# gaurav00700/Selfsupervised-NVSF

Hardware: AMD Instinct MI355X
Metric: rendered rays/sec (LiDAR+cam) (higher is better)
Workload: dtype f16; 1 GPU; C2: KITTI-360 seq-1908-shaped frame per GPU, uniform sampling, static hash field; num_rays=4096, num_rays_lidar=4096, num_steps=768, hash_grid=L16 F2 T2^19 base16 max2048, sigma_mlp=32-64-16, heads=lidar 2x(87-64-64-1), rgb 31-64-64-3, parallelism=frame-sharded x1, no collective

## Files before the change

### selfsupervised-nvsf_amd/csrc/common.h

```cpp
#pragma once
#include <hip/hip_runtime.h>
#include <stdint.h>

#define NVSF_API extern "C" __attribute__((visibility("default")))

enum : int {
    NVSF_OK = 0,
    NVSF_ERR_INVALID_ARG = -1,
    NVSF_ERR_UNSUPPORTED = -2,
};

#define REQUIRE(cond) do { if (!(cond)) return NVSF_ERR_INVALID_ARG; } while (0)

constexpr int kWave = 64;

static inline int nvsf_launch_status() {
    hipError_t e = hipGetLastError();
    return e == hipSuccess ? NVSF_OK : (int)e;
}

static inline unsigned cdiv(unsigned long long a, unsigned b) { return (unsigned)((a + b - 1) / b); }

enum NvsfVariantKey : int {
    kVarMarch = 0,
    kVarPlanesFwd,
    kVarPlanesBwd,
    kVarHashgridFwd,
    kVarHashgridBwd,
    kVarHash4dBwd,
    kVarSlicePlan,
    kVarRenderTail,
    kVarMarchSkew,
    kVarMlpBwd,
    kVarLevelKinds,
    kVarCornerShare,
    kVarCount
};
int nvsf_variant(int key);
int nvsf_cu_count();

__device__ __forceinline__ int lane_id() { return (int)(threadIdx.x & 63); }

__device__ __forceinline__ uint32_t lane_swap(uint32_t v) {
    return (uint32_t)__builtin_amdgcn_mov_dpp((int)v, 0xB1 , 0xF, 0xF, true);
}
__device__ __forceinline__ float lane_swap_f(float v) { return __builtin_bit_cast(float, lane_swap(__builtin_bit_cast(uint32_t, v))); }

template <typename T>
__device__ __forceinline__ T wave_sum(T v) {
#pragma unroll
    for (int o = 32; o > 0; o >>= 1) v += __shfl_xor(v, o, 64);
    return v;
}

__device__ __forceinline__ float wave_scan_add(float v) {
    const int l = lane_id();
#pragma unroll
    for (int o = 1; o < 64; o <<= 1) {
        float u = __shfl_up(v, o, 64);
        if (l >= o) v += u;
    }
    return v;
}
__device__ __forceinline__ float wave_scan_mul(float v) {
    const int l = lane_id();
#pragma unroll
    for (int o = 1; o < 64; o <<= 1) {
        float u = __shfl_up(v, o, 64);
        if (l >= o) v *= u;
    }
    return v;
}
__device__ __forceinline__ uint32_t wave_scan_add_u32(uint32_t v) {
    const int l = lane_id();
#pragma unroll
    for (int o = 1; o < 64; o <<= 1) {
        uint32_t u = __shfl_up(v, o, 64);
        if (l >= o) v += u;
    }
    return v;
}

__device__ __forceinline__ uint32_t wave_scan_max_u32(uint32_t v) {
#define NVSF_DPP_MAX(ctrl, row_mask)                                                                                        \
    {                                                                                                                      \
        const uint32_t u = (uint32_t)__builtin_amdgcn_update_dpp(0, (int)v, ctrl, row_mask, 0xF, false);                   \
        v = u > v ? u : v;                                                                                                 \
    }
    NVSF_DPP_MAX(0x111, 0xF)
    NVSF_DPP_MAX(0x112, 0xF)
    NVSF_DPP_MAX(0x114, 0xF)
    NVSF_DPP_MAX(0x118, 0xF)
    NVSF_DPP_MAX(0x142, 0xA)
    NVSF_DPP_MAX(0x143, 0xC)
#undef NVSF_DPP_MAX
    return v;
}
```

### selfsupervised-nvsf_amd/csrc/fused_field.hip

```cpp
#include "hashgrid_device.h"
#include "mlp_device.h"
#include "encodings_device.h"
#include "march_device.h"
#pragma clang diagnostic ignored "-Wpass-failed"
#include <stdlib.h>

namespace {
constexpr int kBlock = 256;
constexpr int kWavesPerBlock = kBlock / kWave;

struct RayBatch {
    const float* rays_o;
    const float* rays_d;
    const float* nears;
    const float* fars;
    const float* lin;
    const float* noise;
    float lo[3], hi[3];
    float inv_extent;
    float bound;
    uint32_t N, T;
};

__device__ __forceinline__ float sample_z(const RayBatch& rb, float near, float range, float lin, const float* noise) {
// ... 50 lines not shown
        const float near = rb.nears[n], range = rb.fars[n] - near;
        float x[3];
        const float z = sample_point(rb, rb.rays_o + 3 * (size_t)n, rb.rays_d + 3 * (size_t)n, near, range, rb.lin[i], rb.noise + s, x);
        half8_t xf;
#pragma unroll
        for (int q = 0; q < kLevelsPerGroup; ++q) {
            const int l = g * kLevelsPerGroup + q;
            float acc[F];
            encode_level<3, F>(x, table, meta.scale[l], meta.res[l], meta.offset[l], meta.offset[l + 1] - meta.offset[l], acc);
#pragma unroll
            for (int f = 0; f < F; ++f) xf[q * F + f] = (_Float16)acc[f];
        }
        float4_t acc1[kHidTiles];
#pragma unroll
        for (int t = 0; t < kHidTiles; ++t) {
            const float4_t zero = {0, 0, 0, 0};
            acc1[t] = mfma16(w0[t], xf, zero);
        }
        half8_t h[kHidSteps];
        pack_hidden(acc1, h);
        const float4_t o = wout.apply(h);
        if (in_range) {
            half4_t ov;
            ov[0] = (_Float16)o[0]; ov[1] = (_Float16)o[1]; ov[2] = (_Float16)o[2]; ov[3] = (_Float16)o[3];
            if (g == 3) {
                z_vals[s] = z;
                sigmas[s] = expf(o[3]);
                ov[3] = (_Float16)1.0f;
            }
            *reinterpret_cast<half4_t*>(geo + s * 16 + 4 * g) = ov;
        }
    }
}

template <int F>
struct LaneLevels {
    static constexpr int Q = 8 / F;
    float scale[Q];
    uint32_t res[Q], res2[Q], boff[Q], rows[Q];
};

__device__ __forceinline__ void fma_entry(float w, uint32_t raw, float& a0, float& a1) {
    asm("v_fma_mix_f32 %0, %1, %2, %0 op_sel_hi:[0,1,0]" : "+v"(a0) : "v"(w), "v"(raw));
    asm("v_fma_mix_f32 %0, %1, %2, %0 op_sel:[0,1,0] op_sel_hi:[0,1,0]" : "+v"(a1) : "v"(w), "v"(raw));
}

template <int F>
__device__ __forceinline__ uint32_t gather_raw(__amdgpu_buffer_rsrc_t rsrc, uint32_t byte_off);
template <>
__device__ __forceinline__ uint32_t gather_raw<2>(__amdgpu_buffer_rsrc_t rsrc, uint32_t byte_off) {
    return __builtin_amdgcn_raw_buffer_load_b32(rsrc, byte_off, 0, 0);
}
typedef uint32_t entry4_t __attribute__((ext_vector_type(2)));
template <int F> struct EntryOf { typedef uint32_t type; };
template <> struct EntryOf<4> { typedef entry4_t type; };
template <>
__device__ __forceinline__ uint32_t gather_raw<4>(__amdgpu_buffer_rsrc_t, uint32_t) = delete;
__device__ __forceinline__ entry4_t gather_raw4(__amdgpu_buffer_rsrc_t rsrc, uint32_t byte_off) {
    return __builtin_amdgcn_raw_buffer_load_b64(rsrc, byte_off, 0, 0);
}

template <int F>
struct DensityCtx {
    static constexpr int Q = 8 / F;
    LaneLevels<F> lv;
    half8_t w0[kHidTiles];
    OutLayerW wout;
    __amdgpu_buffer_rsrc_t rsrc;
    uint32_t first_hashed;
    int g;
    const uint4* lds_lv;
    uint32_t share_mask;
    uint32_t* share_lds;
};

template <int N>
__device__ __forceinline__ uint32_t row_lane(uint32_t v) {
    return (uint32_t)__builtin_amdgcn_update_dpp(0, (int)v, 0x150 + N, 0xF, 0xF, false);
}

constexpr uint32_t kFirstHashedC2 = 5;
constexpr float kShareLambdaMax = 2.0f;
constexpr int kShareWords = 2 * kWave;
template <int F, int QG, bool LDS_LV = false, int FH = -1, bool SHARE = false>
__device__ __forceinline__ half8_t density_encode(const DensityCtx<F>& cx, const float (&x)[3]) {
    constexpr int Q = 8 / F;
    static_assert(!SHARE || (F == 2 && QG == Q), "the shared form exchanges one dword per lane and runs behind the gathers of all groups");
    LaneLevels<F> lv_local;
    if constexpr (LDS_LV) {
        uint32_t again = 0;
        asm volatile("" : "+v"(again));
#pragma unroll
        for (int q = 0; q < Q; ++q) {
            const uint4 v = cx.lds_lv[4 * q + again];
            lv_local.scale[q] = __builtin_bit_cast(float, v.x);
            lv_local.res[q] = v.y;
            lv_local.res2[q] = v.y * v.y;
            lv_local.boff[q] = v.z;
            lv_local.rows[q] = v.w;
        }
    }
    const LaneLevels<F>& lv = LDS_LV ? lv_local : cx.lv;
    const uint32_t first_hashed = FH >= 0 ? (uint32_t)FH : cx.first_hashed;
    const int g = cx.g;
    half8_t xf;
#pragma unroll
    for (int q0 = 0; q0 < Q; q0 += QG) {
    float frac[Q][3];
    typename EntryOf<F>::type raw[Q][8];
    bool shared[2] = {false, false};
    uint32_t share_sel[2] = {0u, 0u}, share_one[2] = {0u, 0u};
#pragma unroll
    for (int q = q0; q < q0 + QG; ++q) {
        uint32_t c[3];
#pragma unroll
        for (int d = 0; d < 3; ++d) {
            const float pos = fmaf(lv.scale[q], x[d], 0.5f);
            const float fl = floorf(pos);
            frac[q][d] = pos - fl;
            c[d] = (uint32_t)(int32_t)fl;
        }
        const bool all_dense = (uint32_t)(4 * q + 3) < first_hashed, all_hashed = (uint32_t)(4 * q) >= first_hashed;
        if constexpr (SHARE) {
            if (q < 2 && ((cx.share_mask >> q) & 1u)) {
                uint32_t a[3], b[3];
#pragma unroll
                for (int d = 0; d < 3; ++d) {
                    a[d] = row_lane<0>(c[d]);
                    b[d] = row_lane<15>(c[d]);
                }
                const bool in_a = c[0] == a[0] && c[1] == a[1] && c[2] == a[2], in_b = c[0] == b[0] && c[1] == b[1] && c[2] == b[2];
                share_sel[q] = in_a ? 0u : 8u;
                shared[q] = __ballot(!(in_a || in_b)) == 0;
                if (shared[q]) {
                    const uint32_t col = (uint32_t)lane_id() & 15u;
                    const bool of_a = col < 8u;
                    const uint32_t cc[3] = {(of_a ? a[0] : b[0]) + (col & 1u), (of_a ? a[1] : b[1]) + ((col >> 1) & 1u), (of_a ? a[2] : b[2]) + ((col >> 2) & 1u)};
                    uint32_t v = 0;
                    if (all_dense || !all_hashed) {
                        v = cc[0] + cc[1] * lv.res[q] + cc[2] * lv.res2[q];
                        v = v >= lv.rows[q] ? v - lv.rows[q] : v;
                    }
                    if (all_hashed || !all_dense) {
                        const uint32_t h = (cc[0] ^ (cc[1] * 2654435761u) ^ (cc[2] * 805459861u)) & (lv.rows[q] - 1u);
                        v = (all_hashed || (uint32_t)(4 * q + g) >= first_hashed) ? h : v;
                    }
                    share_one[q] = gather_raw<2>(cx.rsrc, lv.boff[q] + v * (uint32_t)(F * sizeof(_Float16)));
                }
            }
        }
        if (!SHARE || q >= 2 || !shared[q]) {
        uint32_t idx[8];
        if (all_dense || !all_hashed) {
            const uint32_t b00 = c[0] + c[1] * lv.res[q] + c[2] * lv.res2[q];
            const uint32_t b10 = b00 + lv.res[q], b01 = b00 + lv.res2[q], b11 = b10 + lv.res2[q];
            const uint32_t base[4] = {b00, b10, b01, b11};
#pragma unroll
            for (int k = 0; k < 8; ++k) {
                uint32_t v = base[k >> 1] + (uint32_t)(k & 1);
                v = v >= lv.rows[q] ? v - lv.rows[q] : v;
                idx[k] = v;
            }
        }
        if (all_hashed || !all_dense) {
            const uint32_t hy0 = c[1] * 2654435761u, hy1 = hy0 + 2654435761u;
            const uint32_t hz0 = c[2] * 805459861u, hz1 = hz0 + 805459861u;
            const uint32_t yz[4] = {hy0 ^ hz0, hy1 ^ hz0, hy0 ^ hz1, hy1 ^ hz1};
            const uint32_t mask = lv.rows[q] - 1u;
            const bool lane_hashed = (uint32_t)(4 * q + g) >= first_hashed;
#pragma unroll
            for (int k = 0; k < 8; ++k) {
                const uint32_t v = ((c[0] + (uint32_t)(k & 1)) ^ yz[k >> 1]) & mask;
                idx[k] = (all_hashed || lane_hashed) ? v : idx[k];
            }
        }
#pragma unroll
        for (int k = 0; k < 8; ++k) {
            if constexpr (F == 2) raw[q][k] = gather_raw<2>(cx.rsrc, lv.boff[q] + idx[k] * (uint32_t)(F * sizeof(_Float16)));
            else raw[q][k] = gather_raw4(cx.rsrc, lv.boff[q] + idx[k] * (uint32_t)(F * sizeof(_Float16)));
        }
        }
    }
    auto blend = [&](int q, const typename EntryOf<F>::type (&r)[8]) {
        const float fx = frac[q][0], fy = frac[q][1], fz = frac[q][2];
        const float wx[2] = {1.0f - fx, fx}, wy[2] = {1.0f - fy, fy}, wz[2] = {1.0f - fz, fz};
        if constexpr (F == 2) {
            float a0 = 0.0f, a1 = 0.0f;
#pragma unroll
            for (int k = 0; k < 8; ++k) {
                const float w = (wx[k & 1] * wy[(k >> 1) & 1]) * wz[k >> 2];
                fma_entry(w, r[k], a0, a1);
            }
            xf[q * F] = (_Float16)a0;
            xf[q * F + 1] = (_Float16)a1;
        } else {
            float a0 = 0.0f, a1 = 0.0f, a2 = 0.0f, a3 = 0.0f;
#pragma unroll
            for (int k = 0; k < 8; ++k) {
                const float w = (wx[k & 1] * wy[(k >> 1) & 1]) * wz[k >> 2];
                fma_entry(w, r[k][0], a0, a1);
                fma_entry(w, r[k][1], a2, a3);
            }
            xf[q * F] = (_Float16)a0;
            xf[q * F + 1] = (_Float16)a1;
            xf[q * F + 2] = (_Float16)a2;
            xf[q * F + 3] = (_Float16)a3;
        }
    };
    if constexpr (SHARE) {
#pragma unroll
        for (int q = 0; q < 2; ++q) {
            if (shared[q]) {
                uint32_t* slot = cx.share_lds + q * kWave;
                slot[lane_id()] = share_one[q];
                const uint4* cell = reinterpret_cast<const uint4*>(slot + 16 * g + share_sel[q]);
                const uint4 lo = cell[0], hi = cell[1];
                const uint32_t r[8] = {lo.x, lo.y, lo.z, lo.w, hi.x, hi.y, hi.z, hi.w};
                blend(q, r);
            } else {
                blend(q, raw[q]);
            }
        }
    }
#pragma unroll
    for (int q = (SHARE ? 2 : q0); q < q0 + QG; ++q) blend(q, raw[q]);
    }
    return xf;
}

template <int F, int QG>
__device__ __forceinline__ float4_t density_eval(const DensityCtx<F>& cx, const float (&x)[3]) {
    const half8_t xf = density_encode<F, QG>(cx, x);
    float4_t acc1[kHidTiles];
#pragma unroll
    for (int t = 0; t < kHidTiles; ++t) {
        const float4_t zero = {0, 0, 0, 0};
        acc1[t] = mfma16(cx.w0[t], xf, zero);
    }
    half8_t h[kHidSteps];
    pack_hidden(acc1, h);
    return cx.wout.apply(h);
}

struct TrainOut {
    float* x01;
    _Float16* feat;
    float* h32;
    uint32_t* tile;
};

__device__ __forceinline__ void store_h32(float* __restrict__ h32, unsigned long long s, int lane, int g, float o0, float o1, float o2, float o3, bool ok) {
    const int from = (lane + 48) & 63;
    const float prev = __int_as_float(__builtin_amdgcn_ds_bpermute(from << 2, __float_as_int(o3)));
    if (ok) *reinterpret_cast<float4*>(h32 + s * 16 + 4 * g) = make_float4(prev, o0, o1, o2);
}

constexpr int kTrPitch = 20;
constexpr int kTrWords = 16 * kTrPitch;
__device__ __forceinline__ void store_feat_row(_Float16* __restrict__ feat, unsigned long long s, int lane, int g, const uint4& p, bool ok,
                                               uint32_t* tile) {
    uint32_t* row = tile + (lane & 15) * kTrPitch;
    row[g] = p.x; row[4 + g] = p.y; row[8 + g] = p.z; row[12 + g] = p.w;
    const uint4 mine = *reinterpret_cast<const uint4*>(row + 4 * g);
    if (ok) *reinterpret_cast<uint4*>(feat + s * 32 + 8 * g) = mine;
}

__device__ __forceinline__ void store_feat_row_swap(_Float16* __restrict__ feat, unsigned long long s, int g, const uint4& p, bool ok) {
    const auto a = __builtin_amdgcn_permlane16_swap(p.x, p.y, false, false);
    const auto b = __builtin_amdgcn_permlane16_swap(p.z, p.w, false, false);
    const auto lo = __builtin_amdgcn_permlane32_swap(a[0], b[0], false, false);
    const auto hi = __builtin_amdgcn_permlane32_swap(a[1], b[1], false, false);
    if (ok) *reinterpret_cast<uint4*>(feat + s * 32 + 8 * g) = make_uint4(lo[0], hi[0], lo[1], hi[1]);
}

template <int F, int QG, bool TRAIN = false>
__device__ __forceinline__ void density_tile(const DensityCtx<F>& cx, const float (&x)[3], float z, unsigned long long s, bool in_range,
                                             float* __restrict__ z_vals, float* __restrict__ sigmas, _Float16* __restrict__ geo,
                                             const TrainOut* tr = nullptr) {
    const int g = cx.g;
    float4_t o;
    if constexpr (TRAIN) {
        const half8_t xf = density_encode<F, QG>(cx, x);
        float4_t acc1[kHidTiles];
#pragma unroll
        for (int t = 0; t < kHidTiles; ++t) {
            const float4_t zero = {0, 0, 0, 0};
            acc1[t] = mfma16(cx.w0[t], xf, zero);
        }
        half8_t h[kHidSteps];
        pack_hidden(acc1, h);
        o = cx.wout.apply(h);
        const int lane = lane_id();
        store_feat_row(tr->feat, s, lane, g, __builtin_bit_cast(uint4, xf), in_range, tr->tile);
        store_h32(tr->h32, s, lane, g, o[0], o[1], o[2], o[3], in_range);
        if (in_range && g == 0) { tr->x01[3 * s] = x[0]; tr->x01[3 * s + 1] = x[1]; tr->x01[3 * s + 2] = x[2]; }
    } else {
        o = density_eval<F, QG>(cx, x);
    }
    if (in_range) {
        half4_t ov;
        ov[0] = (_Float16)o[0]; ov[1] = (_Float16)o[1]; ov[2] = (_Float16)o[2]; ov[3] = (_Float16)o[3];
        if (g == 3) {
            z_vals[s] = z;
            sigmas[s] = expf(o[3]);
            ov[3] = (_Float16)1.0f;
        }
        *reinterpret_cast<half4_t*>(geo + s * 16 + 4 * g) = ov;
    }
}

// ... 88 lines not shown
    float scale;
    uint32_t res, res2, boff, rows;
    bool hashed;
};

template <int F>
__device__ __forceinline__ void slice_issue(const SliceLevel<F>& lv, __amdgpu_buffer_rsrc_t rsrc, const float (&x)[3], float (&frac)[3],
                                            uint32_t (&raw)[8]) {
    uint32_t c[3];
#pragma unroll
    for (int d = 0; d < 3; ++d) {
        const float pos = fmaf(lv.scale, x[d], 0.5f);
        const float fl = floorf(pos);
        frac[d] = pos - fl;
        c[d] = (uint32_t)(int32_t)fl;
    }
    uint32_t idx[8];
    if (!lv.hashed) {
        const uint32_t b00 = c[0] + c[1] * lv.res + c[2] * lv.res2;
        const uint32_t b10 = b00 + lv.res, b01 = b00 + lv.res2, b11 = b10 + lv.res2;
        const uint32_t base[4] = {b00, b10, b01, b11};
#pragma unroll
        for (int k = 0; k < 8; ++k) {
            uint32_t v = base[k >> 1] + (uint32_t)(k & 1);
            idx[k] = v >= lv.rows ? v - lv.rows : v;
        }
    } else {
        const uint32_t hy0 = c[1] * 2654435761u, hy1 = hy0 + 2654435761u;
        const uint32_t hz0 = c[2] * 805459861u, hz1 = hz0 + 805459861u;
        const uint32_t yz[4] = {hy0 ^ hz0, hy1 ^ hz0, hy0 ^ hz1, hy1 ^ hz1};
        const uint32_t mask = lv.rows - 1u;
#pragma unroll
        for (int k = 0; k < 8; ++k) idx[k] = ((c[0] + (uint32_t)(k & 1)) ^ yz[k >> 1]) & mask;
    }
#pragma unroll
    for (int k = 0; k < 8; ++k) raw[k] = gather_raw<F>(rsrc, lv.boff + idx[k] * (uint32_t)(F * sizeof(_Float16)));
}

__device__ __forceinline__ uint32_t slice_blend(const float (&frac)[3], const uint32_t (&raw)[8]) {
    const float fx = frac[0], fy = frac[1], fz = frac[2];
    const float wx[2] = {1.0f - fx, fx}, wy[2] = {1.0f - fy, fy}, wz[2] = {1.0f - fz, fz};
    float a0 = 0.0f, a1 = 0.0f;
#pragma unroll
    for (int k = 0; k < 8; ++k) {
        const float w = (wx[k & 1] * wy[(k >> 1) & 1]) * wz[k >> 2];
        fma_entry(w, raw[k], a0, a1);
    }
    h2_t o;
    o[0] = (_Float16)a0;
    o[1] = (_Float16)a1;
    return __builtin_bit_cast(uint32_t, o);
}

template <int F>
__device__ __forceinline__ void slice_issue_half(const SliceLevel<F>& lv, __amdgpu_buffer_rsrc_t rsrc, const float (&x)[3], uint32_t xb,
                                                 float (&frac)[3], uint32_t (&raw)[4]) {
    uint32_t c[3];
#pragma unroll
    for (int d = 0; d < 3; ++d) {
        const float pos = fmaf(lv.scale, x[d], 0.5f);
        const float fl = floorf(pos);
        frac[d] = pos - fl;
        c[d] = (uint32_t)(int32_t)fl;
    }
    uint32_t idx[4];
    if (!lv.hashed) {
        const uint32_t b00 = c[0] + c[1] * lv.res + c[2] * lv.res2;
        const uint32_t base[4] = {b00, b00 + lv.res, b00 + lv.res2, b00 + lv.res + lv.res2};
#pragma unroll
        for (int p = 0; p < 4; ++p) {
            const uint32_t v = base[p] + xb;
            idx[p] = v >= lv.rows ? v - lv.rows : v;
        }
    } else {
        const uint32_t hy0 = c[1] * 2654435761u, hy1 = hy0 + 2654435761u;
        const uint32_t hz0 = c[2] * 805459861u, hz1 = hz0 + 805459861u;
        const uint32_t yz[4] = {hy0 ^ hz0, hy1 ^ hz0, hy0 ^ hz1, hy1 ^ hz1};
        const uint32_t mask = lv.rows - 1u;
#pragma unroll
        for (int p = 0; p < 4; ++p) idx[p] = ((c[0] + xb) ^ yz[p]) & mask;
    }
#pragma unroll
    for (int p = 0; p < 4; ++p) raw[p] = gather_raw<F>(rsrc, lv.boff + idx[p] * (uint32_t)(F * sizeof(_Float16)));
}

constexpr int kPlanItems = 3;
struct SlicePlan {
    uint32_t n[8];
    uint32_t slice[8][kPlanItems], begin[8][kPlanItems], end[8][kPlanItems];
};

struct EncodeUnit {
    uint32_t s, n;
    bool in_range;
    float near, far, lin, noise, o[3], d[3];
};

template <bool UNIFORM_RAY>
__device__ __forceinline__ EncodeUnit fetch_unit(const RayBatch& rb, uint32_t M, uint32_t half_lane, uint32_t unit, uint32_t n_u, uint32_t i_u) {
    EncodeUnit u;
    const uint32_t s_raw = unit * 32u + half_lane;
    uint32_t i;
    if constexpr (UNIFORM_RAY) {
        u.in_range = true;
        u.s = s_raw;
        u.n = n_u;
        i = i_u + half_lane;
    } else {
        u.in_range = s_raw < M;
        u.s = u.in_range ? s_raw : M - 1u;
        u.n = u.s / rb.T;
        i = u.s - u.n * rb.T;
    }
    u.near = rb.nears[u.n];
    u.far = rb.fars[u.n];
    u.lin = rb.lin[i];
    u.noise = rb.noise ? rb.noise[u.s] : 0.5f;
    load_ray(rb, u.n, u.o, u.d);
    return u;
}

template <bool UNIFORM_RAY>
struct UnitCursor {
    uint32_t ray = 0, first = 0, d_ray = 0, d_first = 0;
    __device__ __forceinline__ UnitCursor(uint32_t wave, uint32_t wave_count, uint32_t T) {
        if constexpr (UNIFORM_RAY) {
            ray = (wave * 32u) / T;
            first = wave * 32u - ray * T;
            d_ray = (wave_count * 32u) / T;
            d_first = wave_count * 32u - d_ray * T;
        }
    }
    __device__ __forceinline__ void advance(uint32_t T) {
        if constexpr (UNIFORM_RAY) {
            ray += d_ray;
            first += d_first;
            if (first >= T) {
                first -= T;
                ray += 1u;
            }
        }
    }
};

template <int F, bool UNIFORM_RAY>
__global__ __launch_bounds__(kBlock) __attribute__((amdgpu_waves_per_eu(8, 8))) void k_encode_sliced_pairs(RayBatch rb, const _Float16* __restrict__ table, uint32_t table_bytes,
                                                                GridMeta meta, uint32_t L, uint32_t first_hashed, uint32_t M,
                                                                float* __restrict__ z_vals, uint2* __restrict__ feat, SlicePlan plan,
                                                                float* __restrict__ x01 = nullptr) {
    static_assert(F == 2, "F = 2 only");
    const uint32_t group = blockIdx.x & 7u, sb = blockIdx.x >> 3, n_sb = gridDim.x >> 3;
    for (uint32_t item = 0; item < plan.n[group]; ++item) {
    const uint32_t slice = plan.slice[group][item], unit_begin = plan.begin[group][item], unit_end = plan.end[group][item];
    const uint32_t grp = slice >> 1;
    const uint32_t lvl[2] = {(slice & 1u) ? grp + 4u : grp, (slice & 1u) ? grp + 8u : grp + 12u};
    SliceLevel<F> lv[2];
#pragma unroll
    for (int a = 0; a < 2; ++a) {
        const uint32_t l = lvl[a];
        lv[a].scale = meta.scale[l];
        lv[a].res = meta.res[l];
        lv[a].res2 = meta.res[l] * meta.res[l];
        lv[a].boff = meta.offset[l] * (uint32_t)(F * sizeof(_Float16));
        lv[a].rows = meta.offset[l + 1] - meta.offset[l];
        lv[a].hashed = l >= first_hashed;
    }
// ... 637 lines not shown
            c[0] = sigmoid_f32(oa[0]); c[1] = sigmoid_f32(oa[1]); c[2] = sigmoid_f32(oa[2]);
        }
#pragma unroll
        for (int i = 0; i < 16; ++i) {
            if ((uint32_t)i < cnt && alive) {
                const float s_i = readlane_f32(sigma, 48 + i);
                const float dt_i = readlane_f32(sdt, i), d1_i = readlane_f32(sd1, i);
                const float alpha = 1.0f - expf(-s_i * dt_i);
                const float T = 1.0f - ws;
                const float w = alpha * T;
                ws += w;
                t_comp += d1_i;
                dep += w * t_comp;
#pragma unroll
                for (int k = 0; k < 3; ++k) col[k] += w * readlane_f32(c[k], i);
                if (T < T_thresh) alive = false;
            }
        }
        total += cnt;
        if (cnt < 16u) alive = false;
    }
    if (lane == 0) {
        weights_sum[n] = ws;
        depth[n] = dep;
        if constexpr (LIDAR) {
            image[2 * (size_t)n] = col[0];
            image[2 * (size_t)n + 1] = col[1];
        } else {
            const float rest = 1.0f - ws;
            image[3 * (size_t)n] = col[0] + rest * bg0;
            image[3 * (size_t)n + 1] = col[1] + rest * bg1;
            image[3 * (size_t)n + 2] = col[2] + rest * bg2;
        }
    }
}

template <int N>
__device__ __forceinline__ float row_shr(float old, float v) {
    static_assert(N >= 1 && N <= 15, "row_shr:1..15");
    return __builtin_bit_cast(float, __builtin_amdgcn_update_dpp(__builtin_bit_cast(int, old), __builtin_bit_cast(int, v), 0x110 + N, 0xF, 0xF, false));
}

__device__ __forceinline__ float row_shl1(float old, float v) {
    return __builtin_bit_cast(float, __builtin_amdgcn_update_dpp(__builtin_bit_cast(int, old), __builtin_bit_cast(int, v), 0x101, 0xF, 0xF, false));
}

__device__ __forceinline__ float row_first(float v) {
    return __builtin_bit_cast(float, __builtin_amdgcn_update_dpp(0, __builtin_bit_cast(int, v), 0x150, 0xF, 0xF, false));
}

__device__ __forceinline__ float row16_scan_mul(float v) {
    v *= row_shr<1>(1.0f, v);
    v *= row_shr<2>(1.0f, v);
    v *= row_shr<4>(1.0f, v);
    v *= row_shr<8>(1.0f, v);
    return v;
}

template <int C>
__device__ __forceinline__ void store_ray(int lane, float ws, float dp, float (&img)[C], float bg0, float bg1, float bg2, int use_bg,
                                          float* __restrict__ weights_sum, float* __restrict__ depth, float* __restrict__ image) {
    ws = wave_sum(ws);
    dp = wave_sum(dp);
#pragma unroll
    for (int k = 0; k < C; ++k) img[k] = wave_sum(img[k]);
    if (lane == 0) {
        *weights_sum = ws;
        *depth = dp;
        const float bg[3] = {bg0, bg1, bg2};
        const float rest = use_bg ? 1.0f - ws : 0.0f;
#pragma unroll
        for (int k = 0; k < C; ++k) image[k] = use_bg ? img[k] + rest * bg[k] : img[k];
    }
}

struct RenderTrainOut {
    float* x01;
    _Float16* feat;
    _Float16* geo;
    float* sigma;
    float* rgb;
};

template <bool LIDAR, bool FROM_FEATURES, bool TRAIN = false, int FH = -1>
__global__ __launch_bounds__(kBlock) __attribute__((amdgpu_waves_per_eu(4, 4))) void k_render_uniform(
    RayBatch rb, const _Float16* __restrict__ table, uint32_t table_bytes, GridMeta meta, uint32_t first_hashed,
    const uint2* __restrict__ feat, const _Float16* __restrict__ w_sigma, const _Float16* __restrict__ w_a, const _Float16* __restrict__ w_b,
    float k_scale, float w_thresh, float bg0, float bg1, float bg2, int use_bg, float* __restrict__ z_vals, float* __restrict__ weights,
    float* __restrict__ weights_sum, float* __restrict__ depth, float* __restrict__ image, float share_thresh = -1.0f,
    RenderTrainOut rt = RenderTrainOut()) {
    using FR = OccFrags<LIDAR>;
    constexpr int F = 2;
    constexpr int IN_STEPS = FR::IN_STEPS;
    constexpr int C = LIDAR ? 2 : 3;
    __shared__ uint4 s_lv[kMaxLevels];
    __shared__ half8_t s_frag[FR::kCount * kWave];
    __shared__ float4_t s_pre[kWavesPerBlock * FR::kPre];
    __shared__ __attribute__((aligned(16))) uint32_t s_share[FROM_FEATURES ? 1 : kWavesPerBlock * kShareWords];
    fill_level_table<F>(s_lv, meta);
    const int lane = lane_id(), g = lane >> 4, c = lane & 15;
    for (int f = (int)(threadIdx.x >> 6); f < FR::kCount; f += kWavesPerBlock) s_frag[f * kWave + lane] = occ_fragment<LIDAR>(f, lane, w_sigma, w_a, w_b);
    __syncthreads();
    const uint32_t n = __builtin_amdgcn_readfirstlane(blockIdx.x * kWavesPerBlock + (threadIdx.x >> 6));
    if (n >= rb.N) return;
    const half8_t* frag = s_frag + lane;
    const uint32_t T = rb.T;
    const size_t M = (size_t)rb.N * T;

    DensityCtx<F> cx;
    if constexpr (!FROM_FEATURES) {
        cx.g = g;
        cx.first_hashed = first_hashed;
        cx.lds_lv = s_lv + g;
        cx.rsrc = __builtin_amdgcn_make_buffer_rsrc(const_cast<_Float16*>(table), 0, (int)table_bytes, 0x00020000);
    }
    const float rd0 = rb.rays_d[3 * (size_t)n], rd1 = rb.rays_d[3 * (size_t)n + 1], rd2 = rb.rays_d[3 * (size_t)n + 2];
    const float d0 = (rd0 + 1.0f) / 2.0f, d1 = (rd1 + 1.0f) / 2.0f, d2 = (rd2 + 1.0f) / 2.0f;
    half8_t xf[IN_STEPS];
    encode_ray_direction<LIDAR>(d0, d1, d2, g, xf);
    const GeoRoute<LIDAR> route(g, lane & 15);
    float4_t* pre = s_pre + (threadIdx.x >> 6) * FR::kPre;
    ray_head_constants<LIDAR>(xf, w_a, w_b, lane, pre);

    const float near = rb.nears[n], range = rb.fars[n] - near;
    const float sample_dist = range / (float)T;
    const float ro[3] = {rb.rays_o[3 * (size_t)n], rb.rays_o[3 * (size_t)n + 1], rb.rays_o[3 * (size_t)n + 2]}, rd[3] = {rd0, rd1, rd2};
    if constexpr (!FROM_FEATURES) {
        const float step1 = (sample_dist * rb.inv_extent) * ((fabsf(rd0) + fabsf(rd1)) + fabsf(rd2));
        const uint32_t m = ((16.0f * meta.scale[3]) * step1 <= share_thresh ? 1u : 0u) | ((16.0f * meta.scale[7]) * step1 <= share_thresh ? 2u : 0u);
        cx.share_mask = __builtin_amdgcn_readfirstlane(m);
        cx.share_lds = s_share + (threadIdx.x >> 6) * kShareWords;
    }
    const size_t row0 = (size_t)n * T;
    float carry = 1.0f, ws = 0.0f, dp = 0.0f, img[C];
#pragma unroll
    for (int k = 0; k < C; ++k) img[k] = 0.0f;
    float lin_cur = 0.0f, lin_nxt = 0.0f, nz_cur = 0.5f, nz_nxt = 0.5f;
    auto request = [&](uint32_t i0) {
        const uint32_t i = i0 + (uint32_t)c;
        const uint32_t ic = i < T ? i : T - 1u, in = ic + 1u < T ? ic + 1u : ic;
        lin_cur = rb.lin[ic];
        lin_nxt = rb.lin[in];
        if (rb.noise) {
            nz_cur = rb.noise[row0 + ic];
            nz_nxt = rb.noise[row0 + in];
        }
    };
    if constexpr (!FROM_FEATURES) request(0u);
    for (uint32_t i0 = 0; i0 < T; i0 += 16) {
        const uint32_t i = i0 + (uint32_t)c;
        const bool valid = i < T;
        const uint32_t ic = valid ? i : T - 1u;
        const size_t s = row0 + ic;
        float z, z_next;
        half8_t feat8;
        if constexpr (FROM_FEATURES) {
            z = z_vals[s];
            z_next = ic + 1u < T ? z_vals[s + 1] : z;
            const uint2 p0 = feat[(size_t)(2 * g) * M + s], p1 = feat[(size_t)(2 * g + 1) * M + s];
            typedef uint32_t u4_t __attribute__((ext_vector_type(4)));
            const u4_t packed = {p0.x, p1.x, p1.y, p0.y};
            feat8 = __builtin_bit_cast(half8_t, packed);
        } else {
            z = sample_z(rb, near, range, lin_cur, &nz_cur);
            z_next = sample_z(rb, near, range, lin_nxt, &nz_nxt);
            if (i0 + 16u < T) request(i0 + 16u);
            float x[3];
            sample_x01(rb, ro, rd, z, x);
            feat8 = density_encode<F, 4, true, FH, true>(cx, x);
            if constexpr (TRAIN) {
                if (g == 0 && valid) { rt.x01[3 * s] = x[0]; rt.x01[3 * s + 1] = x[1]; rt.x01[3 * s + 2] = x[2]; }
            }
        }
        if constexpr (TRAIN) store_feat_row_swap(rt.feat, s, g, __builtin_bit_cast(uint4, feat8), valid);
        const float4_t o = sigma_tile<LIDAR>(frag, feat8);
        const float delta = (i + 1u < T) ? z_next - z : sample_dist;
        float alpha = 0.0f;
        if (g == 3 && valid) alpha = 1.0f - expf(-delta * k_scale * expf(o[3]));
        const float om = (g == 3 && valid) ? (1.0f - alpha + 1e-15f) : 1.0f;
        const float incl = row16_scan_mul(om);
        const float excl = row_shr<1>(1.0f, incl);
        const float w = alpha * (carry * excl);
        carry = carry * readlane_f32(incl, 63);
        if (g == 3 && valid) {
            weights[s] = w;
            if constexpr (!FROM_FEATURES) z_vals[s] = z;
            if constexpr (TRAIN) rt.sigma[s] = expf(o[3]);
        }
        ws += w;
        dp += w * z;
        const float w0 = __shfl(w, 48 + c, 64);
        const bool on = w0 > w_thresh;
        float cr[C];
#pragma unroll
        for (int k = 0; k < C; ++k) cr[k] = 0.0f;
        if constexpr (TRAIN) {
            if (valid) *reinterpret_cast<uint2*>(rt.geo + s * 16 + 4 * g) = make_uint2(pack_h2(o[0], o[1]), pack_h2(o[2], g == 3 ? 1.0f : o[3]));
        }
        if (__ballot(w > w_thresh)) {
            const half8_t x_last = route.apply(o, g, 0, xf[IN_STEPS - 1]);
            const float4_t oa = head_tile<LIDAR>(frag, pre, g, 0, x_last);
            if constexpr (LIDAR) {
                const float4_t ob = head_tile<LIDAR>(frag, pre, g, 1, x_last);
                if (g == 0 && on) {
                    cr[0] = sigmoid_f32(oa[0]);
                    cr[1] = sigmoid_f32(ob[0]);
                    img[0] += w0 * cr[0];
                    img[1] += w0 * cr[1];
                }
            } else {
                if (g == 0 && on) {
#pragma unroll
                    for (int k = 0; k < 3; ++k) {
                        cr[k] = sigmoid_f32(oa[k]);
                        img[k] += w0 * cr[k];
                    }
                }
            }
        }
        if constexpr (TRAIN) {
            if (g == 0 && valid) {
#pragma unroll
                for (int k = 0; k < C; ++k) rt.rgb[s * C + k] = cr[k];
            }
        }
    }
    store_ray<C>(lane, ws, dp, img, bg0, bg1, bg2, use_bg, weights_sum + n, depth + n, image + (size_t)n * C);
}

template <bool LIDAR, bool TRAIN = false>
__global__ __launch_bounds__(kBlock) __attribute__((amdgpu_waves_per_eu(4, 4))) void k_render_tail2(
    RayBatch rb, const uint2* __restrict__ feat, const _Float16* __restrict__ w_sigma, const _Float16* __restrict__ w_a,
    const _Float16* __restrict__ w_b, float k_scale, float w_thresh, float bg0, float bg1, float bg2, int use_bg,
    const float* __restrict__ z_vals, float* __restrict__ weights, float* __restrict__ weights_sum, float* __restrict__ depth,
    float* __restrict__ image, RenderTrainOut rt = RenderTrainOut()) {
    using FR = OccFrags<LIDAR>;
    constexpr int IN_STEPS = FR::IN_STEPS;
    constexpr int C = LIDAR ? 2 : 3;
    constexpr int kOut1 = FR::kCount;
    __shared__ half8_t s_frag[(FR::kCount + kHidSteps) * kWave];
    __shared__ float4_t s_pre[kWavesPerBlock * FR::kPre];
    const int lane = lane_id(), g = lane >> 4, c = lane & 15;
    for (int f = (int)(threadIdx.x >> 6); f < FR::kCount + kHidSteps; f += kWavesPerBlock)
        s_frag[f * kWave + lane] = f < FR::kCount ? occ_fragment<LIDAR>(f, lane, w_sigma, w_a, w_b) : load_w_chained(w_sigma + kHidden * 32, 0, f - FR::kCount, lane, 5);
    __syncthreads();
    const uint32_t n = __builtin_amdgcn_readfirstlane(blockIdx.x * kWavesPerBlock + (threadIdx.x >> 6));
    if (n >= rb.N) return;
    const half8_t* frag = s_frag + lane;
    const uint32_t T = rb.T;
    const size_t M = (size_t)rb.N * T;

    const float rd0 = rb.rays_d[3 * (size_t)n], rd1 = rb.rays_d[3 * (size_t)n + 1], rd2 = rb.rays_d[3 * (size_t)n + 2];
// ... 319 lines not shown
    if (N == 0) return NVSF_OK;
    REQUIRE(T > 0 && weights && geo_f16 && rays_d && head_a_weights_f16 && image);
    REQUIRE(!lidar || head_b_weights_f16);
    REQUIRE(!h_bg_color || weights_sum);
    REQUIRE((reinterpret_cast<uintptr_t>(geo_f16) & 15u) == 0 && (reinterpret_cast<uintptr_t>(head_a_weights_f16) & 15u) == 0 &&
            (reinterpret_cast<uintptr_t>(head_b_weights_f16) & 15u) == 0);
    const _Float16* gp = reinterpret_cast<const _Float16*>(geo_f16);
    const _Float16* wa = reinterpret_cast<const _Float16*>(head_a_weights_f16);
    const _Float16* wb = reinterpret_cast<const _Float16*>(head_b_weights_f16);
    const float b0 = h_bg_color ? h_bg_color[0] : 0.0f, b1 = h_bg_color ? h_bg_color[1] : 0.0f,
                b2 = (h_bg_color && !lidar) ? h_bg_color[2] : 0.0f;
    const dim3 grid(cdiv(N, kWavesPerBlock)), block(kBlock);
    if (lidar)
        hipLaunchKernelGGL(k_heads_uniform<true>, dim3(grid.x, 2), block, 0, stream, weights, gp, rays_d, weights_sum, wa, wb, N, T, w_thresh, b0,
                           b1, b2, h_bg_color ? 1 : 0, image);
    else
        hipLaunchKernelGGL(k_heads_uniform<false>, grid, block, 0, stream, weights, gp, rays_d, weights_sum, wa, wb, N, T, w_thresh,
                           b0, b1, b2, h_bg_color ? 1 : 0, image);
    return nvsf_launch_status();
}

NVSF_API int nvsf_render_occupancy_fwd(const float* rays_o, const float* rays_d, const float* nears, const float* fars,
                                       const uint8_t* grid, float bound, float dt_gamma, uint32_t max_steps, uint32_t C, uint32_t H,
                                       uint32_t N, const void* table_f16, uint32_t L, uint32_t F, const float* h_scales,
                                       const uint32_t* h_res, const uint32_t* h_offsets, const void* sigma_weights_f16, int lidar,
                                       const void* head_a_weights_f16, const void* head_b_weights_f16, float density_scale,
                                       float T_thresh, const float* h_bg_color, float* weights_sum, float* depth, float* image,
                                       hipStream_t stream) {
    if (N == 0) return NVSF_OK;
    REQUIRE(rays_o && rays_d && nears && fars && grid && table_f16 && sigma_weights_f16 && head_a_weights_f16 && weights_sum && depth && image);
    REQUIRE(!lidar || head_b_weights_f16);
    REQUIRE(bound > 0.0f && C >= 1 && C <= 8 && H >= 2 && H <= 1024 && max_steps >= 1);
    REQUIRE((reinterpret_cast<uintptr_t>(table_f16) & 15u) == 0 && (reinterpret_cast<uintptr_t>(sigma_weights_f16) & 15u) == 0 &&
            (reinterpret_cast<uintptr_t>(head_a_weights_f16) & 15u) == 0 && (reinterpret_cast<uintptr_t>(head_b_weights_f16) & 15u) == 0);
    if ((F != 2 && F != 4) || L * F != 32) return NVSF_ERR_UNSUPPORTED;
    GridInfo gi;
    const int st = classify_grid(gi, L, F, h_scales, h_res, h_offsets);
    if (st != NVSF_OK) return st;
    if (!gi.dense_first || gi.table_bytes >= (1ull << 31)) return NVSF_ERR_UNSUPPORTED;
    OccRays rr;
    rr.rays_o = rays_o; rr.rays_d = rays_d; rr.nears = nears; rr.fars = fars; rr.grid = grid;
    rr.bound = bound; rr.dt_gamma = dt_gamma; rr.max_steps = max_steps; rr.C = C; rr.H = H; rr.N = N;
    const FieldParams w(table_f16, sigma_weights_f16, head_a_weights_f16, head_b_weights_f16, h_bg_color);
    const dim3 grid_dim(cdiv(N, kWavesPerBlock)), block(kBlock);
#define LAUNCH_OCC(LD, FF, FH)                                                                                                            \
    hipLaunchKernelGGL((k_render_occupancy_lds<LD, FF, FH>), grid_dim, block, 0, stream, rr, w.table, (uint32_t)gi.table_bytes, gi.meta,       \
                       gi.first_hashed, w.sigma, w.head_a, w.head_b, density_scale, T_thresh, w.bg[0], w.bg[1], w.bg[2], weights_sum, depth, \
                       image)
    const bool c2_grid = F == 2 && gi.first_hashed == kFirstHashedC2 && nvsf_variant(kVarLevelKinds) == 0;
    if (lidar) { if (c2_grid) LAUNCH_OCC(true, 2, (int)kFirstHashedC2); else if (F == 2) LAUNCH_OCC(true, 2, -1); else LAUNCH_OCC(true, 4, -1); }
    else { if (c2_grid) LAUNCH_OCC(false, 2, (int)kFirstHashedC2); else if (F == 2) LAUNCH_OCC(false, 2, -1); else LAUNCH_OCC(false, 4, -1); }
#undef LAUNCH_OCC
    return nvsf_launch_status();
}

static int render_uniform_impl(const float* rays_o, const float* rays_d, const float* nears, const float* fars, const float* lin,
                               const float* noise, const float* h_aabb, float bound, uint32_t N, uint32_t T, const void* table_f16,
                               uint32_t L, uint32_t F, const float* h_scales, const uint32_t* h_res, const uint32_t* h_offsets,
                               const void* sigma_weights_f16, int lidar, const void* head_a_weights_f16,
                               const void* head_b_weights_f16, float k_scale, float w_thresh, const float* h_bg_color,
                               const void* feat_scratch, float* z_vals, float* weights, float* weights_sum, float* depth, float* image,
                               hipStream_t stream, const RenderTrainOut* train) {
    if (N == 0 || T == 0) return NVSF_OK;
    REQUIRE(rays_o && rays_d && nears && fars && h_aabb && table_f16 && sigma_weights_f16 && head_a_weights_f16);
    REQUIRE(z_vals && weights && weights_sum && depth && image && (feat_scratch || lin));
    REQUIRE(!lidar || head_b_weights_f16);
    REQUIRE(bound > 0.0f);
    REQUIRE((reinterpret_cast<uintptr_t>(table_f16) & 15u) == 0 && (reinterpret_cast<uintptr_t>(sigma_weights_f16) & 15u) == 0 &&
            (reinterpret_cast<uintptr_t>(head_a_weights_f16) & 15u) == 0 && (reinterpret_cast<uintptr_t>(head_b_weights_f16) & 15u) == 0 &&
            (reinterpret_cast<uintptr_t>(feat_scratch) & 15u) == 0);
    if (!((F == 2 && L == 16) || (F == 4 && L == 8 && feat_scratch))) return NVSF_ERR_UNSUPPORTED;
    GridInfo gi;
    const int st = classify_grid(gi, L, F, h_scales, h_res, h_offsets);
    if (st != NVSF_OK) return st;
    if (!gi.dense_first || gi.table_bytes >= (1ull << 31)) return NVSF_ERR_UNSUPPORTED;
    const RayBatch rb = make_ray_batch(rays_o, rays_d, nears, fars, lin, noise, h_aabb, bound, N, T);
    const FieldParams w(table_f16, sigma_weights_f16, head_a_weights_f16, head_b_weights_f16, h_bg_color);
    const uint2* fp = reinterpret_cast<const uint2*>(feat_scratch);
    const RenderTrainOut rt = train ? *train : RenderTrainOut();
    const int use_bg = (h_bg_color && !lidar) ? 1 : 0;
    const dim3 grid_dim(cdiv(N, kWavesPerBlock)), block(kBlock);
    const int cs = nvsf_variant(kVarCornerShare);
    const float share_thresh = cs == 1 ? -1.0f : cs == 2 ? INFINITY : kShareLambdaMax;
#define LAUNCH_RU_FH(LD, FF, FH)                                                                                                      \
    do {                                                                                                                              \
        if (train)                                                                                                                    \
            hipLaunchKernelGGL((k_render_uniform<LD, FF, true, FH>), grid_dim, block, 0, stream, rb, w.table, (uint32_t)gi.table_bytes, gi.meta, \
                               gi.first_hashed, fp, w.sigma, w.head_a, w.head_b, k_scale, w_thresh, w.bg[0], w.bg[1], w.bg[2], use_bg, z_vals,   \
                               weights, weights_sum, depth, image, share_thresh, rt);                                                               \
        else                                                                                                                          \
            hipLaunchKernelGGL((k_render_uniform<LD, FF, false, FH>), grid_dim, block, 0, stream, rb, w.table, (uint32_t)gi.table_bytes, gi.meta, \
                               gi.first_hashed, fp, w.sigma, w.head_a, w.head_b, k_scale, w_thresh, w.bg[0], w.bg[1], w.bg[2], use_bg, z_vals,    \
                               weights, weights_sum, depth, image, share_thresh, rt);                                                               \
    } while (0)
#define LAUNCH_RU(LD, FF)                                                                                                             \
    do {                                                                                                                              \
        if (!FF && gi.first_hashed == kFirstHashedC2 && nvsf_variant(kVarLevelKinds) == 0) LAUNCH_RU_FH(LD, FF, (FF ? -1 : (int)kFirstHashedC2)); \
        else LAUNCH_RU_FH(LD, FF, -1);                                                                                                \
    } while (0)
#define LAUNCH_TAIL(LD)                                                                                                               \
    do {                                                                                                                              \
        if (train)                                                                                                                    \
            hipLaunchKernelGGL((k_render_tail2<LD, true>), grid_dim, block, 0, stream, rb, fp, w.sigma, w.head_a, w.head_b, k_scale, w_thresh, \
                               w.bg[0], w.bg[1], w.bg[2], use_bg, z_vals, weights, weights_sum, depth, image, rt);                    \
        else                                                                                                                          \
            hipLaunchKernelGGL((k_render_tail2<LD, false>), grid_dim, block, 0, stream, rb, fp, w.sigma, w.head_a, w.head_b, k_scale, w_thresh, \
                               w.bg[0], w.bg[1], w.bg[2], use_bg, z_vals, weights, weights_sum, depth, image, rt);                    \
    } while (0)
    const bool tail2 = nvsf_variant(kVarRenderTail) == 0;
    if (lidar) { if (fp) { if (tail2) LAUNCH_TAIL(true); else LAUNCH_RU(true, true); } else LAUNCH_RU(true, false); }
    else { if (fp) { if (tail2) LAUNCH_TAIL(false); else LAUNCH_RU(false, true); } else LAUNCH_RU(false, false); }
#undef LAUNCH_TAIL
#undef LAUNCH_RU
#undef LAUNCH_RU_FH
    return nvsf_launch_status();
}

NVSF_API int nvsf_render_uniform_fwd(const float* rays_o, const float* rays_d, const float* nears, const float* fars, const float* lin,
                                     const float* noise, const float* h_aabb, float bound, uint32_t N, uint32_t T, const void* table_f16,
                                     uint32_t L, uint32_t F, const float* h_scales, const uint32_t* h_res, const uint32_t* h_offsets,
                                     const void* sigma_weights_f16, int lidar, const void* head_a_weights_f16,
                                     const void* head_b_weights_f16, float k_scale, float w_thresh, const float* h_bg_color,
                                     const void* feat_scratch, float* z_vals, float* weights, float* weights_sum, float* depth, float* image,
                                     hipStream_t stream) {
    return render_uniform_impl(rays_o, rays_d, nears, fars, lin, noise, h_aabb, bound, N, T, table_f16, L, F, h_scales, h_res, h_offsets,
                               sigma_weights_f16, lidar, head_a_weights_f16, head_b_weights_f16, k_scale, w_thresh, h_bg_color, feat_scratch,
                               z_vals, weights, weights_sum, depth, image, stream, nullptr);
}

NVSF_API int nvsf_render_uniform_train_fwd(const float* rays_o, const float* rays_d, const float* nears, const float* fars, const float* lin,
                                           const float* noise, const float* h_aabb, float bound, uint32_t N, uint32_t T,
                                           const void* table_f16, uint32_t L, uint32_t F, const float* h_scales, const uint32_t* h_res,
                                           const uint32_t* h_offsets, const void* sigma_weights_f16, int lidar,
                                           const void* head_a_weights_f16, const void* head_b_weights_f16, float k_scale, float w_thresh,
                                           const float* h_bg_color, void* feat_scratch, float* z_vals, float* weights, float* weights_sum,
                                           float* depth, float* image, float* x01, void* feat_rows_f16, void* geo_f16, float* sigmas,
                                           float* rgbs, hipStream_t stream) {
    if (N == 0 || T == 0) return NVSF_OK;
    REQUIRE(x01 && feat_rows_f16 && geo_f16 && sigmas && rgbs && lin);
    REQUIRE((reinterpret_cast<uintptr_t>(feat_rows_f16) & 15u) == 0 && (reinterpret_cast<uintptr_t>(geo_f16) & 15u) == 0);
    RenderTrainOut rt;
    rt.x01 = x01; rt.feat = reinterpret_cast<_Float16*>(feat_rows_f16); rt.geo = reinterpret_cast<_Float16*>(geo_f16);
    rt.sigma = sigmas; rt.rgb = rgbs;
    if (feat_scratch) {
        TrainOut tr;
        tr.x01 = x01; tr.feat = rt.feat; tr.h32 = nullptr; tr.tile = nullptr;
        const int st = density_uniform_impl(rays_o, rays_d, nears, fars, lin, noise, h_aabb, bound, N, T, table_f16, L, F, h_scales, h_res, h_offsets,
                                            sigma_weights_f16, z_vals, sigmas, geo_f16, feat_scratch, 1u, stream, &tr);
        if (st != NVSF_OK) return st;
    }
    return render_uniform_impl(rays_o, rays_d, nears, fars, lin, noise, h_aabb, bound, N, T, table_f16, L, F, h_scales, h_res, h_offsets,
                               sigma_weights_f16, lidar, head_a_weights_f16, head_b_weights_f16, k_scale, w_thresh, h_bg_color, feat_scratch,
                               z_vals, weights, weights_sum, depth, image, stream, &rt);
}
```

### selfsupervised-nvsf_amd/csrc/version.hip

```cpp
#include "common.h"
#include <string.h>
NVSF_API const char* nvsf_version(void) { return "nvsf_hip 0.1.0 gfx950"; }

#ifndef NVSF_CSRC_DIGEST_ALL
#define NVSF_CSRC_DIGEST_ALL "unknown_________"
#endif
#ifndef NVSF_CSRC_DIGEST_RENDER
#define NVSF_CSRC_DIGEST_RENDER "unknown_________"
#endif
#define NVSF_MARK_ALL "NVSF_CSRC_DIGEST_ALL="
#define NVSF_MARK_RENDER "NVSF_CSRC_DIGEST_RENDER="
static const char g_digest_all[] = NVSF_MARK_ALL NVSF_CSRC_DIGEST_ALL;
static const char g_digest_render[] = NVSF_MARK_RENDER NVSF_CSRC_DIGEST_RENDER;
NVSF_API const char* nvsf_build_digest(int which) {
    return which == 1 ? g_digest_render + sizeof(NVSF_MARK_RENDER) - 1 : g_digest_all + sizeof(NVSF_MARK_ALL) - 1;
}

static int g_variant[kVarCount] = {};
__attribute__((visibility("hidden"))) int nvsf_variant(int key) { return key >= 0 && key < kVarCount ? g_variant[key] : 0; }

__attribute__((visibility("hidden"))) int nvsf_cu_count() {
    static const int n = [] {
        int dev = 0, v = 0;
        if (hipGetDevice(&dev) != hipSuccess || hipDeviceGetAttribute(&v, hipDeviceAttributeMultiprocessorCount, dev) != hipSuccess || v <= 0) v = 256;
        return v;
    }();
    return n;
}

NVSF_API int nvsf_test_variant(const char* name, int value) {
    static const char* const names[kVarCount] = {"march", "planes_fwd", "planes_bwd", "hashgrid_fwd", "hashgrid_bwd", "hash4d_bwd", "slice_plan",
                                                 "render_tail", "march_skew", "mlp_bwd", "level_kinds", "corner_share"};
    if (!name || value < 0) return NVSF_ERR_INVALID_ARG;
    for (int k = 0; k < kVarCount; ++k)
        if (strcmp(name, names[k]) == 0) {
            const int old = g_variant[k];
            g_variant[k] = value;
            return old;
        }
    return NVSF_ERR_INVALID_ARG;
}
```

### selfsupervised-nvsf_amd/nvsf/testing.py

```python
import contextlib

_NATIVE = {
    "march": {"wave": 0, "thread": 1, "serial": 2},
    "planes_fwd": {"runs": 0, "sample": 1},
    "planes_bwd": {"runs": 0, "atomic": 1, "global": 2},
    "hashgrid_fwd": {"auto": 0, "generic": 1},
    "hashgrid_bwd": {"corners": 0, "atomic": 1},
    "hash4d_bwd": {"lds": 0, "runs": 1},
    "slice_plan": {"balanced": 0, "home": 1},
    "render_tail": {"two": 0, "one": 1},
    "mlp_bwd": {"auto": 0, "staged": 1, "wave": 2},
    "level_kinds": {"compiled": 0, "runtime": 1},
    "corner_share": {"gated": 0, "never": 1, "always": 2},
    "march_skew": {"off": 0, **{f"queue{q}": q + 1 for q in range(8)}},
}
_PYTHON = {
    "heads_input": ("prefix", "rows"),
    "density_sliced": (None, False, True),
    "hash4d_train": ("fused", "slices"),
    "dynamic_fused": (True, False),
    "density_tail_train": ("fused", "chain"),
    "density_fn": ("fused", "chain"),
    "planes_train": ("fused", "separate"),
    "density_grad": ("composed", "matrix"),
    "hash4d_scatter": ("side", "main"),
    "table_scatter": ("binned", "atomic"),
}
_state = {}


def get(name):
    return _state.get(name, _PYTHON[name][0])


@contextlib.contextmanager
def variant(**choices):
    from nvsf import _hip
    lib = _hip.load()
    undo_native, undo_python = [], []
    try:
        for name, value in choices.items():
            if name in _NATIVE:
                code = _NATIVE[name][value]
                old = lib.nvsf_test_variant(name.encode(), code)
                if old < 0:
                    raise _hip.NvsfHipError(f"nvsf_test_variant({name!r}) rejected")
                undo_native.append((name, old))
            elif name in _PYTHON:
                if value not in _PYTHON[name]:
                    raise ValueError(f"{name}: one of {_PYTHON[name]}")
                undo_python.append((name, _state.get(name, _PYTHON[name][0])))
                _state[name] = value
            else:
                raise KeyError(name)
        yield
    finally:
        for name, old in reversed(undo_native):
            lib.nvsf_test_variant(name.encode(), old)
        for name, old in reversed(undo_python):
            _state[name] = old
```

Baseline: 12.92 million rays/s.

## Pair lanes to split fine hash-level corner gathers across x-halves

Adds a paired-gather path for the fine levels (q>=2) of the shared density encoder in the uniform render kernel. Each lane pair now issues half of the corner gathers for two levels, split by x-bit, using a sample position redistributed via bpermute. The halves are swapped with a DPP lane swap, blended, and routed back to the owning lane with ds_bpermute. The aim is better coalescing and fewer scattered gather instructions per lane, at the cost of extra cross-lane traffic, more address math and more register pressure. It is enabled by default for non-feature launches and can be turned off through a new variant switch.

Result: slower. 12.49 million rays/s (-3.3%).

```diff
diff --git a/selfsupervised-nvsf_amd/csrc/common.h b/selfsupervised-nvsf_amd/csrc/common.h
--- a/selfsupervised-nvsf_amd/csrc/common.h
+++ b/selfsupervised-nvsf_amd/csrc/common.h
@@ -34,6 +34,7 @@
     kVarMlpBwd,
     kVarLevelKinds,
     kVarCornerShare,
+    kVarPairGather,
     kVarCount
 };
 int nvsf_variant(int key);
diff --git a/selfsupervised-nvsf_amd/csrc/fused_field.hip b/selfsupervised-nvsf_amd/csrc/fused_field.hip
--- a/selfsupervised-nvsf_amd/csrc/fused_field.hip
+++ b/selfsupervised-nvsf_amd/csrc/fused_field.hip
@@ -156,10 +156,17 @@
 constexpr uint32_t kFirstHashedC2 = 5;
 constexpr float kShareLambdaMax = 2.0f;
 constexpr int kShareWords = 2 * kWave;
-template <int F, int QG, bool LDS_LV = false, int FH = -1, bool SHARE = false>
-__device__ __forceinline__ half8_t density_encode(const DensityCtx<F>& cx, const float (&x)[3]) {
+template <int F> struct SliceLevel;
+template <int F>
+__device__ void slice_issue_half(const SliceLevel<F>& lv, __amdgpu_buffer_rsrc_t rsrc, const float (&x)[3], uint32_t xb, float (&frac)[3], uint32_t (&raw)[4]);
+__device__ void pair_exchange(uint32_t xb, const uint32_t (&half_raw)[2][4], uint32_t (&raw)[8]);
+__device__ uint32_t slice_blend(const float (&frac)[3], const uint32_t (&raw)[8]);
+
+template <int F, int QG, bool LDS_LV = false, int FH = -1, bool SHARE = false, bool PAIR = false>
+__device__ __forceinline__ half8_t density_encode(const DensityCtx<F>& cx, const float (&x)[3], const float (&xp)[3]) {
     constexpr int Q = 8 / F;
     static_assert(!SHARE || (F == 2 && QG == Q), "the shared form exchanges one dword per lane and runs behind the gathers of all groups");
+    static_assert(!PAIR || (SHARE && LDS_LV), "the paired form is the fine half of the shared form's kernels and reads the LDS level table");
     LaneLevels<F> lv_local;
     if constexpr (LDS_LV) {
         uint32_t again = 0;
@@ -184,8 +191,38 @@
     typename EntryOf<F>::type raw[Q][8];
     bool shared[2] = {false, false};
     uint32_t share_sel[2] = {0u, 0u}, share_one[2] = {0u, 0u};
+    const uint32_t pair_xb = (uint32_t)lane_id() & 1u, pair_r = (uint32_t)lane_id() >> 5;
+    float pair_frac[2][3];
+    uint32_t pair_raw[2][2][4];
 #pragma unroll
     for (int q = q0; q < q0 + QG; ++q) {
+        if constexpr (PAIR) {
+            if (q >= 2) {
+                uint32_t again = 0;
+                asm volatile("" : "+v"(again));
+                const uint4* pair_lv = cx.lds_lv + ((int)(2u * pair_r) - g) + 4 * q + again;
+                float fr[2][3], own_scale = 0.0f;
+#pragma unroll
+                for (int a = 0; a < 2; ++a) {
+                    const uint4 v = pair_lv[a];
+                    SliceLevel<F> pl;
+                    pl.scale = __builtin_bit_cast(float, v.x);
+                    own_scale = (uint32_t)a == pair_xb ? pl.scale : own_scale;
+                    pl.res = v.y;
+                    pl.res2 = v.y * v.y;
+                    pl.boff = v.z;
+                    pl.rows = v.w;
+                    pl.hashed = (uint32_t)(4 * q) >= first_hashed || (uint32_t)(4 * q + a) + 2u * pair_r >= first_hashed;
+                    slice_issue_half<F>(pl, cx.rsrc, xp, pair_xb, fr[a], pair_raw[q - 2][a]);
+                }
+#pragma unroll
+                for (int d = 0; d < 3; ++d) {
+                    const float pos = fmaf(own_scale, xp[d], 0.5f);
+                    pair_frac[q - 2][d] = pos - floorf(pos);
+                }
+                continue;
+            }
+        }
         uint32_t c[3];
 #pragma unroll
         for (int d = 0; d < 3; ++d) {
@@ -296,10 +333,30 @@
             }
         }
     }
-#pragma unroll
-    for (int q = (SHARE ? 2 : q0); q < q0 + QG; ++q) blend(q, raw[q]);
+    if constexpr (PAIR) {
+        const int from = ((g >> 1) << 5) | ((lane_id() & 15) << 1) | (g & 1);
+        uint32_t moved[2];
+#pragma unroll
+        for (int j = 0; j < 2; ++j) {
+            uint32_t r[8];
+            pair_exchange(pair_xb, pair_raw[j], r);
+            moved[j] = (uint32_t)__builtin_amdgcn_ds_bpermute(from << 2, (int)slice_blend(pair_frac[j], r));
+        }
+        uint4 packed = __builtin_bit_cast(uint4, xf);
+        packed.z = moved[0];
+        packed.w = moved[1];
+        xf = __builtin_bit_cast(half8_t, packed);
+    } else {
+#pragma unroll
+        for (int q = (SHARE ? 2 : q0); q < q0 + QG; ++q) blend(q, raw[q]);
+    }
     }
     return xf;
+}
+
+template <int F, int QG, bool LDS_LV = false, int FH = -1>
+__device__ __forceinline__ half8_t density_encode(const DensityCtx<F>& cx, const float (&x)[3]) {
+    return density_encode<F, QG, LDS_LV, FH, false, false>(cx, x, x);
 }
 
 template <int F, int QG>
@@ -554,6 +611,17 @@
     }
 #pragma unroll
     for (int p = 0; p < 4; ++p) raw[p] = gather_raw<F>(rsrc, lv.boff + idx[p] * (uint32_t)(F * sizeof(_Float16)));
+}
+
+__device__ __forceinline__ void pair_exchange(uint32_t xb, const uint32_t (&half_raw)[2][4], uint32_t (&raw)[8]) {
+#pragma unroll
+    for (int p = 0; p < 4; ++p) {
+        const uint32_t own = xb ? half_raw[1][p] : half_raw[0][p];
+        const uint32_t send = xb ? half_raw[0][p] : half_raw[1][p];
+        const uint32_t recv = lane_swap(send);
+        raw[2 * p] = xb ? recv : own;
+        raw[2 * p + 1] = xb ? own : recv;
+    }
 }
 
 constexpr int kPlanItems = 3;
@@ -1357,7 +1425,7 @@
     float* rgb;
 };
 
-template <bool LIDAR, bool FROM_FEATURES, bool TRAIN = false, int FH = -1>
+template <bool LIDAR, bool FROM_FEATURES, bool TRAIN = false, int FH = -1, bool PAIR = false>
 __global__ __launch_bounds__(kBlock) __attribute__((amdgpu_waves_per_eu(4, 4))) void k_render_uniform(
     RayBatch rb, const _Float16* __restrict__ table, uint32_t table_bytes, GridMeta meta, uint32_t first_hashed,
     const uint2* __restrict__ feat, const _Float16* __restrict__ w_sigma, const _Float16* __restrict__ w_a, const _Float16* __restrict__ w_b,
@@ -1440,9 +1508,15 @@
             z = sample_z(rb, near, range, lin_cur, &nz_cur);
             z_next = sample_z(rb, near, range, lin_nxt, &nz_nxt);
             if (i0 + 16u < T) request(i0 + 16u);
-            float x[3];
+            float x[3], xp[3];
             sample_x01(rb, ro, rd, z, x);
-            feat8 = density_encode<F, 4, true, FH, true>(cx, x);
+            if constexpr (PAIR) {
+                const float zp = __builtin_bit_cast(float, __builtin_amdgcn_ds_bpermute(((lane >> 1) & 15) << 2, __builtin_bit_cast(int, z)));
+                sample_x01(rb, ro, rd, zp, xp);
+            } else {
+                xp[0] = x[0]; xp[1] = x[1]; xp[2] = x[2];
+            }
+            feat8 = density_encode<F, 4, true, FH, true, PAIR>(cx, x, xp);
             if constexpr (TRAIN) {
                 if (g == 0 && valid) { rt.x01[3 * s] = x[0]; rt.x01[3 * s + 1] = x[1]; rt.x01[3 * s + 2] = x[2]; }
             }
@@ -1928,16 +2002,22 @@
     const dim3 grid_dim(cdiv(N, kWavesPerBlock)), block(kBlock);
     const int cs = nvsf_variant(kVarCornerShare);
     const float share_thresh = cs == 1 ? -1.0f : cs == 2 ? INFINITY : kShareLambdaMax;
-#define LAUNCH_RU_FH(LD, FF, FH)                                                                                                      \
+#define LAUNCH_RU_PP(LD, FF, FH, PP)                                                                                                  \
     do {                                                                                                                              \
         if (train)                                                                                                                    \
-            hipLaunchKernelGGL((k_render_uniform<LD, FF, true, FH>), grid_dim, block, 0, stream, rb, w.table, (uint32_t)gi.table_bytes, gi.meta, \
+            hipLaunchKernelGGL((k_render_uniform<LD, FF, true, FH, PP>), grid_dim, block, 0, stream, rb, w.table, (uint32_t)gi.table_bytes, gi.meta, \
                                gi.first_hashed, fp, w.sigma, w.head_a, w.head_b, k_scale, w_thresh, w.bg[0], w.bg[1], w.bg[2], use_bg, z_vals,   \
                                weights, weights_sum, depth, image, share_thresh, rt);                                                               \
         else                                                                                                                          \
-            hipLaunchKernelGGL((k_render_uniform<LD, FF, false, FH>), grid_dim, block, 0, stream, rb, w.table, (uint32_t)gi.table_bytes, gi.meta, \
+            hipLaunchKernelGGL((k_render_uniform<LD, FF, false, FH, PP>), grid_dim, block, 0, stream, rb, w.table, (uint32_t)gi.table_bytes, gi.meta, \
                                gi.first_hashed, fp, w.sigma, w.head_a, w.head_b, k_scale, w_thresh, w.bg[0], w.bg[1], w.bg[2], use_bg, z_vals,    \
                                weights, weights_sum, depth, image, share_thresh, rt);                                                               \
+    } while (0)
+    const bool pair = nvsf_variant(kVarPairGather) == 0;
+#define LAUNCH_RU_FH(LD, FF, FH)                                                                                                      \
+    do {                                                                                                                              \
+        if (!FF && pair) LAUNCH_RU_PP(LD, FF, FH, !FF);                                                                               \
+        else LAUNCH_RU_PP(LD, FF, FH, false);                                                                                         \
     } while (0)
 #define LAUNCH_RU(LD, FF)                                                                                                             \
     do {                                                                                                                              \
@@ -1959,6 +2039,7 @@
 #undef LAUNCH_TAIL
 #undef LAUNCH_RU
 #undef LAUNCH_RU_FH
+#undef LAUNCH_RU_PP
     return nvsf_launch_status();
 }
 
diff --git a/selfsupervised-nvsf_amd/csrc/version.hip b/selfsupervised-nvsf_amd/csrc/version.hip
--- a/selfsupervised-nvsf_amd/csrc/version.hip
+++ b/selfsupervised-nvsf_amd/csrc/version.hip
@@ -30,7 +30,7 @@
 
 NVSF_API int nvsf_test_variant(const char* name, int value) {
     static const char* const names[kVarCount] = {"march", "planes_fwd", "planes_bwd", "hashgrid_fwd", "hashgrid_bwd", "hash4d_bwd", "slice_plan",
-                                                 "render_tail", "march_skew", "mlp_bwd", "level_kinds", "corner_share"};
+                                                 "render_tail", "march_skew", "mlp_bwd", "level_kinds", "corner_share", "pair_gather"};
     if (!name || value < 0) return NVSF_ERR_INVALID_ARG;
     for (int k = 0; k < kVarCount; ++k)
         if (strcmp(name, names[k]) == 0) {
diff --git a/selfsupervised-nvsf_amd/nvsf/testing.py b/selfsupervised-nvsf_amd/nvsf/testing.py
--- a/selfsupervised-nvsf_amd/nvsf/testing.py
+++ b/selfsupervised-nvsf_amd/nvsf/testing.py
@@ -12,6 +12,7 @@
     "mlp_bwd": {"auto": 0, "staged": 1, "wave": 2},
     "level_kinds": {"compiled": 0, "runtime": 1},
     "corner_share": {"gated": 0, "never": 1, "always": 2},
+    "pair_gather": {"always": 0, "never": 1},
     "march_skew": {"off": 0, **{f"queue{q}": q + 1 for q in range(8)}},
 }
 _PYTHON = {
```
